# PaddlePaddle/Paddle3D

Measured on AMD Instinct MI355X. Metric: scenes/sec CenterPoint-Pillars nuScenes 300k-pt sweeps, higher is better.
Workload: dtype f32

## Files before the change

include/paddle3d_amd.h:

```cpp
#ifndef PADDLE3D_AMD_H
#define PADDLE3D_AMD_H

#include <stddef.h>
#include <stdint.h>

#ifdef __cplusplus
extern "C" {
#endif

#define PD3_OK 0
#define PD3_EINVAL (-1)
#define PD3_EWORKSPACE (-2)
#define PD3_EUNSUPPORTED (-3)

int pd3_version(void);
const char *pd3_target_arch(void);

int pd3_selfcheck_lds_atomic_order(const uint32_t *addr, uint32_t *old, int blocks, int waves_per_block, int rounds,
                                   int table, void *stream);

size_t pd3_hard_voxelize_workspace(int batch, int64_t max_points, int num_point_dim,
                                   const float *voxel_size, const float *point_cloud_range,
                                   int max_num_points_in_voxel, int max_voxels);
int pd3_hard_voxelize(const float *points, const int32_t *num_points, int batch, int64_t max_points,
                      int num_point_dim, const float *voxel_size, const float *point_cloud_range,
                      int max_num_points_in_voxel, int max_voxels, float *voxels, int32_t *coords,
                      int32_t *num_points_per_voxel, int32_t *num_voxels, int32_t *coors_batched,
                      void *workspace, size_t workspace_bytes, void *stream);
int pd3_hard_voxelize_path(const float *points, const int32_t *num_points, int batch, int64_t max_points,
                           int num_point_dim, const float *voxel_size, const float *point_cloud_range,
                           int max_num_points_in_voxel, int max_voxels, float *voxels, int32_t *coords,
                           int32_t *num_points_per_voxel, int32_t *num_voxels, int32_t *coors_batched,
                           void *workspace, size_t workspace_bytes, void *stream, int path);

int64_t pd3_hard_voxelize_index_list_entries(int batch, int64_t max_points);
int pd3_hard_voxelize_index(const float *points, const int32_t *num_points, int batch, int64_t max_points,
                            int num_point_dim, const float *voxel_size, const float *point_cloud_range,
                            int max_num_points_in_voxel, int max_voxels, int32_t *vox_span, int32_t *point_list,
                            int32_t *coords, int32_t *num_points_per_voxel, int32_t *num_voxels,
                            int32_t *coors_batched, void *workspace, size_t workspace_bytes, void *stream);

int pd3_hard_voxelize_f64(const double *points, const int32_t *num_points, int batch, int64_t max_points,
                          int num_point_dim, const float *voxel_size, const float *point_cloud_range,
                          int max_num_points_in_voxel, int max_voxels, double *voxels, int32_t *coords,
                          int32_t *num_points_per_voxel, int32_t *num_voxels, int32_t *coors_batched,
                          void *workspace, size_t workspace_bytes, void *stream);

int pd3_dynamic_voxelize(const float *points, int64_t num_points, int num_point_dim, const float *voxel_size,
                         const float *point_cloud_range, int32_t *coors, void *stream);

size_t pd3_pointpillars_scatter_workspace(int batch, int ny, int nx);
int pd3_pointpillars_scatter(const float *voxel_features, const int32_t *coords,
                             int64_t num_pillars, int channels, int batch, int ny, int nx,
                             float *canvas, void *workspace, size_t workspace_bytes, void *stream);

int pd3_pointpillars_inverse_map(const int32_t *coords, int64_t num_pillars, int batch, int ny, int nx,
                                 int32_t *inv, void *stream);
int pd3_scatter_conv3x3_bias_relu(const float *voxel_features, const int32_t *inv, const float *w_packed,
                                  const float *bias, int batch, int cin, int cout, int ny, int nx, int stride,
                                  int relu, float *out, int out_w, void *stream);

size_t pd3_pillar_conv_rulebook_workspace(int batch, int ny, int nx, int stride);
int pd3_pillar_conv_rulebook(const int32_t *inverse_map, int batch, int ny, int nx, int stride, int32_t *nbr,
                             int32_t *out_cell, int32_t *cell_row, int32_t *n_out, int capacity, int32_t *order,
                             void *workspace, size_t workspace_bytes, void *stream);
int pd3_rows_to_dense_fill(const float *rows, const int32_t *cell_row, const float *fill, int batch, int channels, int h,
                           int w, float *out, void *stream);

int pd3_pillar_feature_net(const float *voxels, const int32_t *num_points, const int32_t *coors,
                           int64_t num_pillars, int max_points, int num_point_dim,
                           int voxel_center_dims, float vx, float vy, float vz, float x_offset,
                           float y_offset, float z_offset, const float *w1, const float *scale1,
                           const float *shift1, int c1, const float *w2, const float *scale2,
                           const float *shift2, int c2, float *out, void *stream);

int pd3_pillar_feature_net_path(const float *voxels, const int32_t *num_points, const int32_t *coors,
                                int64_t num_pillars, int max_points, int num_point_dim,
                                int voxel_center_dims, float vx, float vy, float vz, float x_offset,
                                float y_offset, float z_offset, const float *w1, const float *scale1,
                                const float *shift1, int c1, const float *w2, const float *scale2,
                                const float *shift2, int c2, float *out, int path, void *stream);

int pd3_pillar_feature_net_indexed(const float *points, int64_t points_per_frame, const int32_t *vox_span,
                                   const int32_t *point_list, int64_t list_stride, const int32_t *coors,
                                   int64_t num_pillars, int pillars_per_frame, int max_points, int num_point_dim,
                                   int voxel_center_dims, float vx, float vy, float vz, float x_offset,
                                   float y_offset, float z_offset, const float *w1, const float *scale1,
                                   const float *shift1, int c1, const float *w2, const float *scale2,
                                   const float *shift2, int c2, float *out, void *stream);

int pd3_voxel_mean(const float *voxels, const int32_t *num_points, int64_t num_voxels,
                   int max_points, int num_point_dim, float *out, void *stream);

size_t pd3_nms_workspace(int num_boxes);
int pd3_nms_bev(const float *boxes, int num_boxes, float nms_overlap_thresh, int32_t *keep,
                int32_t *num_to_keep, void *workspace, size_t workspace_bytes, void *stream);
int pd3_nms_normal(const float *boxes, int num_boxes, float nms_overlap_thresh, int32_t *keep,
                   int32_t *num_to_keep, void *workspace, size_t workspace_bytes, void *stream);
int pd3_boxes_iou_bev(const float *boxes_a, int num_a, const float *boxes_b, int num_b,
                      float *ans_iou, void *stream);
int pd3_boxes_overlap_bev(const float *boxes_a, int num_a, const float *boxes_b, int num_b,
                          float *ans_overlap, void *stream);
int pd3_libm_eval(int op, const float *x, const float *y, float *out, int64_t n, void *stream);

size_t pd3_centerpoint_postprocess_workspace(int batch, int num_tasks, int feat_h, int feat_w,
                                             int nms_pre_max_size, int nms_post_max_size);
int pd3_centerpoint_postprocess(const float *const *hm, const float *const *reg,
                                const float *const *height, const float *const *dim,
                                const float *const *vel, const float *const *rot, int batch,
                                int num_tasks, const int *hm_channels, int feat_h, int feat_w,
                                const float *voxel_size, const float *point_cloud_range,
                                const float *post_center_range, const int *label_offsets,
                                int down_ratio, float score_threshold, float nms_iou_threshold,
                                int nms_pre_max_size, int nms_post_max_size, int with_velocity,
                                float *out_bboxes, float *out_scores, int64_t *out_labels,
                                int32_t *out_count, void *workspace, size_t workspace_bytes,
                                void *stream);

int pd3_centerpoint_postprocess_strided(const float *const *hm, const float *const *reg,
                                const float *const *height, const float *const *dim,
                                const float *const *vel, const float *const *rot, int64_t head_batch_stride, int batch,
                                int num_tasks, const int *hm_channels, int feat_h, int feat_w,
                                const float *voxel_size, const float *point_cloud_range,
                                const float *post_center_range, const int *label_offsets,
                                int down_ratio, float score_threshold, float nms_iou_threshold,
                                int nms_pre_max_size, int nms_post_max_size, int with_velocity,
                                float *out_bboxes, float *out_scores, int64_t *out_labels,
                                int32_t *out_count, void *workspace, size_t workspace_bytes,
                                void *stream, int selection);
int pd3_centerpoint_postprocess_records(const float *const *hm, const float *const *reg,
                                        const float *const *height, const float *const *dim,
                                        const float *const *vel, const float *const *rot,
                                        int64_t head_batch_stride, int batch, int num_tasks,
                                        const int *hm_channels, int feat_h, int feat_w, const float *voxel_size,
                                        const float *point_cloud_range, const float *post_center_range,
                                        const int *label_offsets, int down_ratio, float score_threshold,
                                        float nms_iou_threshold, int nms_pre_max_size, int nms_post_max_size,
                                        int with_velocity, float *out_bboxes, float *out_scores,
                                        int64_t *out_labels, int32_t *out_count, float *out_records,
                                        int max_per_img, void *workspace, size_t workspace_bytes, void *stream);

size_t pd3_bevdet_postprocess_workspace(int batch, int num_tasks, const int *task_classes, int feat_h, int feat_w,
                                        int max_num);
int pd3_bevdet_postprocess(const float *const *heatmap, const float *const *reg, const float *const *height,
                           const float *const *dim, const float *const *rot, const float *const *vel, int batch,
                           int num_tasks, const int *task_classes, int feat_h, int feat_w, const int *nms_type,
                           const float *nms_thr, const double *min_radius, const float *rescale_factors,
                           int max_num, int pre_max_size, int post_max_size, float score_threshold, int norm_bbox,
                           const float *post_center_range, const float *post_center_limit_range,
                           const float *pc_range, const float *voxel_size, float out_size_factor,
// ... 310 lines not shown
```

paddle3d_amd/_lib.py:

```python
from __future__ import annotations

import ctypes as C
import os
from functools import lru_cache

_HERE = os.path.dirname(os.path.abspath(__file__))
LIB_PATH = os.path.join(_HERE, "lib", "libpaddle3d_amd.so")

c_f32p = C.c_void_p
c_i32p = C.c_void_p

_SIGNATURES = {
    "pd3_version": (C.c_int, []),
    "pd3_target_arch": (C.c_char_p, []),
    "pd3_hard_voxelize_workspace": (C.c_size_t, [C.c_int, C.c_int64, C.c_int, C.c_void_p, C.c_void_p,
                                                 C.c_int, C.c_int]),
    "pd3_hard_voxelize": (C.c_int, [C.c_void_p, C.c_void_p, C.c_int, C.c_int64, C.c_int, C.c_void_p,
                                    C.c_void_p, C.c_int, C.c_int, C.c_void_p, C.c_void_p, C.c_void_p,
                                    C.c_void_p, C.c_void_p, C.c_void_p, C.c_size_t, C.c_void_p]),
    "pd3_hard_voxelize_f64": (C.c_int, [C.c_void_p, C.c_void_p, C.c_int, C.c_int64, C.c_int, C.c_void_p,
                                    C.c_void_p, C.c_int, C.c_int, C.c_void_p, C.c_void_p, C.c_void_p,
                                    C.c_void_p, C.c_void_p, C.c_void_p, C.c_size_t, C.c_void_p]),
    "pd3_hard_voxelize_path": (C.c_int, [C.c_void_p, C.c_void_p, C.c_int, C.c_int64, C.c_int, C.c_void_p,
                                         C.c_void_p, C.c_int, C.c_int, C.c_void_p, C.c_void_p, C.c_void_p,
# ... 98 lines not shown
    "pd3_gather_gemm_f16": (C.c_int, [C.c_void_p, C.c_void_p, C.c_void_p, C.c_int, C.c_int, C.c_int, C.c_int,
                                      C.c_void_p, C.c_void_p, C.c_void_p, C.c_void_p, C.c_void_p, C.c_int, C.c_void_p,
                                      C.c_void_p, C.c_int, C.c_int, C.c_int, C.c_void_p]),
    "pd3_sparse_tile_order_entries": (C.c_int64, [C.c_int]),
    "pd3_sparse_tile_order": (C.c_int, [C.c_void_p, C.c_void_p, C.c_int, C.c_int, C.c_void_p, C.c_void_p]),
    "pd3_sparse_plan_workspace": (C.c_size_t, [C.c_int]),
    "pd3_sparse_conv_outputs_workspace": (C.c_size_t, [C.c_int] + [C.c_void_p] * 4),
    "pd3_sparse_sort_coords": (C.c_int, [C.c_void_p, C.c_int, C.c_int, C.c_void_p, C.c_void_p, C.c_void_p,
                                         C.c_void_p, C.c_void_p, C.c_size_t, C.c_void_p]),
    "pd3_sparse_conv_outputs": (C.c_int, [C.c_void_p, C.c_void_p, C.c_int, C.c_int, C.c_void_p, C.c_void_p,
                                          C.c_void_p, C.c_void_p, C.c_void_p, C.c_void_p, C.c_int, C.c_void_p,
                                          C.c_size_t, C.c_void_p]),
    "pd3_sparse_rulebook_workspace": (C.c_size_t, [C.c_int, C.c_void_p]),
    "pd3_sparse_rulebook": (C.c_int, [C.c_void_p, C.c_void_p, C.c_int, C.c_void_p, C.c_void_p, C.c_int, C.c_int,
                                      C.c_void_p, C.c_void_p, C.c_void_p, C.c_void_p, C.c_int, C.c_void_p,
                                      C.c_void_p, C.c_void_p, C.c_size_t, C.c_void_p]),
    "pd3_sparse_to_dense": (C.c_int, [C.c_void_p, C.c_void_p, C.c_void_p, C.c_int, C.c_int, C.c_int,
                                      C.c_void_p, C.c_void_p, C.c_void_p]),
    "pd3_selfcheck_lds_atomic_order": (C.c_int, [C.c_void_p, C.c_void_p, C.c_int, C.c_int, C.c_int, C.c_int,
                                                 C.c_void_p]),
    "pd3_conv3x3_f16_bias_relu": (C.c_int, [C.c_void_p, C.c_void_p, C.c_void_p, C.c_int, C.c_int, C.c_int, C.c_int,
                                            C.c_int, C.c_int, C.c_void_p, C.c_int, C.c_int, C.c_void_p]),
    "pd3_f32_nchw_to_f16_nhwc": (C.c_int, [C.c_void_p, C.c_int, C.c_int, C.c_int, C.c_int, C.c_void_p, C.c_void_p]),
    "pd3_conv3x3_f16_bias_relu_dual": (C.c_int, [C.c_void_p, C.c_void_p, C.c_void_p, C.c_int, C.c_int, C.c_int, C.c_int,
                                                 C.c_int, C.c_int, C.c_void_p, C.c_void_p, C.c_int, C.c_void_p]),
    "pd3_conv3x3_s2_f16_bias_relu": (C.c_int, [C.c_void_p, C.c_void_p, C.c_void_p, C.c_int, C.c_int, C.c_int, C.c_int,
                                               C.c_int, C.c_int, C.c_void_p, C.c_void_p]),
    "pd3_scatter_conv3x3_s2_f16_bias_relu": (C.c_int, [C.c_void_p, C.c_void_p, C.c_void_p, C.c_void_p, C.c_int, C.c_int,
                                                       C.c_int, C.c_int, C.c_int, C.c_int, C.c_void_p, C.c_int,
                                                       C.c_void_p]),
    "pd3_grouped_conv3x3_small_f16": (C.c_int, [C.c_void_p, C.c_void_p, C.c_void_p, C.c_int, C.c_int, C.c_int, C.c_int,
                                                C.c_int, C.c_int, C.c_void_p, C.c_int, C.c_int, C.c_void_p]),
    "pd3_grouped_conv3x3_small_f16_gm": (C.c_int, [C.c_void_p, C.c_void_p, C.c_void_p, C.c_int, C.c_int, C.c_int, C.c_int,
                                                   C.c_int, C.c_int, C.c_void_p, C.c_int, C.c_int, C.c_void_p]),
    "pd3_stable_argsort_workspace": (C.c_size_t, [C.c_int64, C.c_uint32]),
    "pd3_stable_argsort": (C.c_int, [C.c_void_p, C.c_int64, C.c_int, C.c_uint32, C.c_void_p, C.c_void_p, C.c_size_t,
                                     C.c_void_p]),
    "pd3_conv3x3_winograd43_pp_bias_relu": (C.c_int, [C.c_void_p, C.c_void_p, C.c_void_p, C.c_int, C.c_int, C.c_int,
                                                       C.c_int, C.c_int, C.c_int, C.c_int, C.c_void_p, C.c_void_p]),
    "pd3_conv3x3_winograd43_pp_trace": (C.c_int, [C.c_void_p, C.c_void_p, C.c_void_p, C.c_int, C.c_int, C.c_int, C.c_int,
                                                  C.c_int, C.c_int, C.c_void_p, C.c_void_p, C.c_void_p]),
    "pd3_merge_sweeps_workspace": (C.c_size_t, [C.c_int64]),
    "pd3_merge_sweeps": (C.c_int, [C.c_void_p, C.c_void_p, C.c_int, C.c_int, C.c_int, C.c_void_p, C.c_void_p,
                                   C.c_void_p, C.c_int, C.c_float, C.c_void_p, C.c_void_p, C.c_void_p, C.c_size_t,
                                   C.c_void_p]),
    "pd3_dynamic_voxelize": (C.c_int, [C.c_void_p, C.c_int64, C.c_int, C.c_void_p, C.c_void_p, C.c_void_p, C.c_void_p]),
    "pd3_conv3x3_bias_relu": (C.c_int, [C.c_void_p, C.c_void_p, C.c_void_p, C.c_int, C.c_int, C.c_int, C.c_int,
                                        C.c_int, C.c_int, C.c_int, C.c_int, C.c_void_p, C.c_int, C.c_void_p]),
    "pd3_conv3x3_winograd_bias_relu": (C.c_int, [C.c_void_p, C.c_void_p, C.c_void_p, C.c_int, C.c_int, C.c_int,
                                                 C.c_int, C.c_int, C.c_int, C.c_void_p, C.c_void_p]),
    "pd3_conv3x3_winograd43_bias_relu": (C.c_int, [C.c_void_p, C.c_void_p, C.c_void_p, C.c_int, C.c_int, C.c_int,
                                                   C.c_int, C.c_int, C.c_int, C.c_int, C.c_void_p, C.c_int,
                                                   C.c_void_p]),
    "pd3_patch_conv_bias_relu": (C.c_int, [C.c_void_p, C.c_void_p, C.c_void_p, C.c_int, C.c_int, C.c_int, C.c_int,
                                           C.c_int, C.c_int, C.c_int, C.c_int, C.c_void_p, C.c_int, C.c_int,
                                           C.c_void_p]),
    "pd3_patch_conv_x3_bias_relu": (C.c_int, [C.c_void_p, C.c_void_p, C.c_void_p, C.c_int, C.c_int, C.c_int, C.c_int,
                                              C.c_int, C.c_int, C.c_int, C.c_int, C.c_void_p, C.c_int, C.c_int,
                                              C.c_void_p]),
    "pd3_conv3x3_s2_x3_bias_relu": (C.c_int, [C.c_void_p, C.c_void_p, C.c_void_p, C.c_int, C.c_int, C.c_int, C.c_int,
                                              C.c_int, C.c_int, C.c_int, C.c_void_p, C.c_int, C.c_void_p]),
    "pd3_winograd43_input_transform_floats": (C.c_size_t, [C.c_int] * 4),
    "pd3_winograd43_input_transform": (C.c_int, [C.c_void_p, C.c_int, C.c_int, C.c_int, C.c_int, C.c_int, C.c_void_p,
                                                 C.c_void_p]),
    "pd3_conv3x3_winograd43_ppv_bias_relu": (C.c_int, [C.c_void_p, C.c_void_p, C.c_void_p, C.c_int, C.c_int, C.c_int,
                                                       C.c_int, C.c_int, C.c_int, C.c_int, C.c_void_p, C.c_void_p]),
    "pd3_ssd_postprocess_workspace": (C.c_size_t, [C.c_int] * 7),
    "pd3_ssd_postprocess": (C.c_int, [C.c_void_p, C.c_int64, C.c_int, C.c_int, C.c_int, C.c_int, C.c_int, C.c_int,
                                      C.c_int, C.c_int, C.c_int, C.c_void_p, C.c_void_p, C.c_void_p, C.c_int64,
                                      C.c_int, C.c_int, C.c_float, C.c_float, C.c_void_p, C.c_float, C.c_int, C.c_int,
                                      C.c_void_p, C.c_void_p, C.c_void_p, C.c_void_p, C.c_void_p, C.c_size_t,
                                      C.c_void_p, C.c_int]),
    "pd3_pointpillars_inverse_map": (C.c_int, [C.c_void_p, C.c_int64, C.c_int, C.c_int, C.c_int, C.c_void_p,
                                               C.c_void_p]),
    "pd3_scatter_conv3x3_bias_relu": (C.c_int, [C.c_void_p, C.c_void_p, C.c_void_p, C.c_void_p, C.c_int, C.c_int,
                                                C.c_int, C.c_int, C.c_int, C.c_int, C.c_int, C.c_void_p, C.c_int,
                                                C.c_void_p]),
    "pd3_pillar_conv_rulebook_workspace": (C.c_size_t, [C.c_int] * 4),
    "pd3_pillar_conv_rulebook": (C.c_int, [C.c_void_p, C.c_int, C.c_int, C.c_int, C.c_int, C.c_void_p, C.c_void_p,
                                           C.c_void_p, C.c_void_p, C.c_int, C.c_void_p, C.c_void_p, C.c_size_t,
                                           C.c_void_p]),
    "pd3_rows_to_dense_fill": (C.c_int, [C.c_void_p, C.c_void_p, C.c_void_p, C.c_int, C.c_int, C.c_int, C.c_int,
                                         C.c_void_p, C.c_void_p]),
    "pd3_bevdet_postprocess_workspace": (C.c_size_t, [C.c_int, C.c_int, C.c_void_p, C.c_int, C.c_int, C.c_int]),
    "pd3_bevdet_postprocess": (C.c_int, [C.c_void_p] * 6 + [C.c_int, C.c_int, C.c_void_p, C.c_int, C.c_int,
                                         C.c_void_p, C.c_void_p, C.c_void_p, C.c_void_p, C.c_int, C.c_int,
                                         C.c_int, C.c_float, C.c_int, C.c_void_p, C.c_void_p, C.c_void_p,
                                         C.c_void_p, C.c_float, C.c_void_p, C.c_void_p, C.c_void_p, C.c_void_p,
                                         C.c_void_p, C.c_size_t, C.c_void_p]),
    "pd3_circle_nms_workspace": (C.c_size_t, [C.c_int]),
    "pd3_circle_nms": (C.c_int, [C.c_void_p, C.c_int, C.c_double, C.c_void_p, C.c_void_p, C.c_void_p, C.c_size_t,
                                 C.c_void_p]),
    "pd3_bevdet4d_align": (C.c_int, [C.c_void_p, C.c_void_p] + [C.c_int] * 6 + [C.c_void_p] * 12),
    "pd3_grouped_conv3x3_small": (C.c_int, [C.c_void_p, C.c_void_p, C.c_void_p, C.c_int, C.c_int, C.c_int, C.c_int,
                                            C.c_int, C.c_int, C.c_void_p, C.c_void_p]),
    "pd3_grouped_conv3x3_small_slice": (C.c_int, [C.c_void_p, C.c_void_p, C.c_void_p, C.c_int, C.c_int, C.c_int,
                                                  C.c_int, C.c_int, C.c_int, C.c_void_p, C.c_int, C.c_int,
                                                  C.c_void_p]),
}

SYMBOLS = tuple(_SIGNATURES)

_SIGNATURES_ROI = {
    "pd3_voxel_pool": (C.c_int, [C.c_void_p] * 8 + [C.c_int] * 7 + [C.c_float] + [C.c_int] * 5 + [C.c_void_p] * 2),
    "pd3_roi_grid_points": (C.c_int, [C.c_void_p, C.c_int64, C.c_int, C.c_int] + [C.c_void_p] * 3 + [C.c_int] +
                            [C.c_void_p] * 3),
    "pd3_rcnn_decode_boxes": (C.c_int, [C.c_void_p, C.c_void_p, C.c_int64, C.c_void_p, C.c_void_p]),
    "pd3_class_agnostic_nms_workspace": (C.c_size_t, [C.c_int, C.c_int64, C.c_int]),
    "pd3_class_agnostic_nms": (C.c_int, [C.c_void_p, C.c_void_p, C.c_int, C.c_int64, C.c_int, C.c_int, C.c_float,
                                         C.c_void_p, C.c_int, C.c_float, C.c_int] + [C.c_void_p] * 5 +
                               [C.c_size_t, C.c_void_p]),
}

SYMBOLS_ROI = tuple(_SIGNATURES_ROI)

_SIGNATURES_HEAD = {
    "pd3_grouped_conv3x3_small_counts_slice": (C.c_int, [C.c_void_p, C.c_void_p, C.c_void_p, C.c_int, C.c_int, C.c_int,
                                                         C.c_int, C.c_void_p, C.c_int, C.c_int, C.c_void_p, C.c_int,
                                                         C.c_int, C.c_void_p]),
}

SYMBOLS_HEAD = tuple(_SIGNATURES_HEAD)

_SIGNATURES_PVRCNN = {
    "pd3_stack_sa_pool": (C.c_int, [C.c_void_p] * 11 + [C.c_int] * 5 + [C.c_float, C.c_int] + [C.c_void_p] * 2),
    "pd3_bev_interpolate": (C.c_int, [C.c_void_p, C.c_void_p, C.c_int64] + [C.c_int] * 4 + [C.c_float] * 5 +
                            [C.c_void_p] * 2),
}

SYMBOLS_PVRCNN = tuple(_SIGNATURES_PVRCNN)

_CADDN_GRID = [C.c_int] * 3 + [C.c_void_p] * 2 + [C.c_int, C.c_double, C.c_double]
_CADDN_IN = [C.c_void_p] * 5 + [C.c_int] * 5 + _CADDN_GRID
_SIGNATURES_CADDN = {
    "pd3_frustum_grid": (C.c_int, [C.c_void_p] * 3 + [C.c_int] + _CADDN_GRID + [C.c_int] + [C.c_void_p] * 2),
    "pd3_frustum_to_voxel_workspace": (C.c_size_t, [C.c_int] * 5),
    "pd3_frustum_to_voxel": (C.c_int, _CADDN_IN + [C.c_void_p, C.c_void_p, C.c_size_t, C.c_void_p]),
    "pd3_frustum_to_bev_workspace": (C.c_size_t, [C.c_int] * 7),
    "pd3_frustum_to_bev": (C.c_int, _CADDN_IN + [C.c_void_p] * 3 + [C.c_int, C.c_void_p, C.c_void_p, C.c_size_t,
                                                                    C.c_void_p]),
}

SYMBOLS_CADDN = tuple(_SIGNATURES_CADDN)

_SIGNATURES_BEVFORMER = {
    "pd3_bevformer_point_sampling": (C.c_int, [C.c_void_p] * 3 + [C.c_int] * 6 + [C.c_void_p] * 5),
    "pd3_bevformer_sca": (C.c_int, [C.c_void_p] * 7 + [C.c_int] * 9 + [C.c_void_p] * 2),
    "pd3_bevformer_tsa": (C.c_int, [C.c_void_p] * 6 + [C.c_int] * 7 + [C.c_void_p] * 2),
}

SYMBOLS_BEVFORMER = tuple(_SIGNATURES_BEVFORMER)

_SIGNATURES_BEVFORMER_DEC = {
    "pd3_mha_forward": (C.c_int, [C.c_void_p] * 3 + [C.c_int] * 5 + [C.c_float] + [C.c_void_p] * 2),
    "pd3_bevformer_dec_ca": (C.c_int, [C.c_void_p] * 6 + [C.c_int] * 8 + [C.c_void_p] * 2),
    "pd3_nms_free_decode": (C.c_int, [C.c_void_p] * 3 + [C.c_int] * 5 + [C.c_double, C.c_int] + [C.c_void_p] * 5),
}

SYMBOLS_BEVFORMER_DEC = tuple(_SIGNATURES_BEVFORMER_DEC)

_SIGNATURES_PETR = {
    "pd3_mha_stream_forward": (C.c_int, [C.c_void_p] * 4 + [C.c_int] * 5 + [C.c_float] + [C.c_void_p] * 2),
    "pd3_petr_coords3d": (C.c_int, [C.c_void_p] + [C.c_int] * 6 + [C.c_double, C.c_void_p, C.c_int] + [C.c_void_p] * 4),
}

SYMBOLS_PETR = tuple(_SIGNATURES_PETR)
# ... 44 lines not shown
```

paddle3d_amd/ops/conv.py:

```python
from __future__ import annotations

import ctypes

import torch

from ._common import check, lib, ptr, require_gpu, stream_ptr

__all__ = ["pack_conv3x3_weight", "conv3x3_bias_relu", "supported", "pitch4", "pack_grouped_weight", "grouped_conv3x3_small",
           "grouped_small_supported", "winograd_supported", "pack_winograd_weight", "conv3x3_winograd_bias_relu",
           "patch_mode", "patch_supported", "pack_patch_weight", "patch_conv_bias_relu",
           "patch_x3_supported", "pack_patch_weight_x3", "patch_conv_x3_bias_relu", "split_bf16x3",
           "conv3x3_s2_x3_supported", "pack_conv3x3_s2_x3_weight", "conv3x3_s2_x3_bias_relu",
           "winograd43_input_transform", "conv3x3_winograd43_ppv_bias_relu",
           "winograd43_supported", "winograd43_tile", "pack_winograd43_weight", "conv3x3_winograd43_bias_relu",
           "WINOGRAD43_PP_MIN_CIN", "winograd43_pp_supported", "pack_winograd43_lane_weight", "conv3x3_winograd43_pp_bias_relu",
           "f16_supported", "f16_tile", "pack_conv3x3_f16_weight", "conv3x3_f16_bias_relu", "to_f16_nhwc",
           "pack_grouped_weight_f16", "grouped_conv3x3_small_f16", "conv3x3_f16_bias_relu_dual",
           "s2_f16_supported", "conv3x3_s2_f16_bias_relu", "scatter_conv_s2_f16_supported",
           "scatter_conv3x3_s2_f16_bias_relu", "scatter_conv_sparse_supported", "scatter_conv3x3_sparse"]


def pitch4(w: int) -> int:
    return (int(w) + 3) // 4 * 4


def supported(cin: int, cout: int, h: int, w: int, stride: int = 1) -> bool:
    return stride in (1, 2) and cin % 8 == 0 and cout % 64 == 0 and h % stride == 0 and w % stride == 0


def pack_conv3x3_weight(weight: torch.Tensor) -> torch.Tensor:
    cout, cin = weight.shape[:2]
    assert weight.shape[2:] == (3, 3) and cout % 64 == 0 and cin % 8 == 0
    w = weight.reshape(cout // 64, 64, cin // 8, 4, 2, 9).permute(0, 2, 3, 5, 4, 1)
    return w.reshape(cout // 64, cin // 8, 72, 64).contiguous()


def conv3x3_bias_relu(x: torch.Tensor, w_packed: torch.Tensor, bias, cout: int, relu: bool = True,
                      stride: int = 1, out: torch.Tensor | None = None, w_valid: int | None = None) -> torch.Tensor:
    xx = require_gpu(x, "conv3x3_bias_relu")
    n, cin, h, w = xx.shape
    wv = w if w_valid is None else int(w_valid)
    if out is None:
        out = torch.empty((n, cout, h // stride, pitch4(wv // stride)), dtype=torch.float32, device=xx.device)
    check(lib().pd3_conv3x3_bias_relu(ptr(xx), ptr(w_packed), ptr(bias), n, cin, cout, h, w, wv, int(stride),
                                      int(bool(relu)), ptr(out), int(out.shape[3]), stream_ptr(xx.device)),
          "conv3x3_bias_relu")
    return out


def scatter_conv_supported(cin: int, cout: int, ny: int, nx: int, stride: int) -> bool:
    return stride == 2 and cin % 8 == 0 and cout % 64 == 0 and ny % 2 == 0 and nx % 2 == 0


def scatter_conv3x3_bias_relu(canvas, w_packed: torch.Tensor, bias, cout: int, relu: bool = True) -> torch.Tensor:
    f, inv = canvas.features, canvas.inv
    n, cin, ny, nx = canvas.shape
    wo = pitch4(nx // 2)
    out = torch.empty((n, cout, ny // 2, wo), dtype=torch.float32, device=f.device)
    check(lib().pd3_scatter_conv3x3_bias_relu(ptr(f), ptr(inv), ptr(w_packed), ptr(bias), n, cin, cout, ny, nx, 2,
                                              int(bool(relu)), ptr(out), wo, stream_ptr(f.device)),
          "scatter_conv3x3_bias_relu")
    return out


def scatter_conv_sparse_supported(cin: int, cout: int, ny: int, nx: int, stride: int) -> bool:
    ho, wo = (ny - 1) // stride + 1, (nx - 1) // stride + 1
    return stride == 2 and cin % 16 == 0 and cout in (64, 128) and wo % 4 == 0 and (ho * wo) % 4 == 0


def scatter_conv3x3_sparse(canvas, weight: torch.Tensor, bias: torch.Tensor, packed=None, relu: bool = True):
    from . import sparse_conv3d as sp
    from ._common import workspace

    f, inv = canvas.features, canvas.inv
    n, cin, ny, nx = canvas.shape
    cout = int(weight.shape[0])
    ho, wo = (ny - 1) // 2 + 1, (nx - 1) // 2 + 1
    cap = n * ho * wo
    dev = f.device
    L = lib()
    nbr = torch.empty((cap, 9), dtype=torch.int32, device=dev)
    out_cell = torch.empty((cap,), dtype=torch.int32, device=dev)
    cell_row = torch.empty((n, ho * wo), dtype=torch.int32, device=dev)
    n_out = torch.empty((1,), dtype=torch.int32, device=dev)
    ws = workspace(L.pd3_pillar_conv_rulebook_workspace(n, ny, nx, 2), dev)
    order = torch.empty((int(L.pd3_sparse_tile_order_entries(cap)),), dtype=torch.int32, device=dev)
    check(L.pd3_pillar_conv_rulebook(ptr(inv), n, ny, nx, 2, ptr(nbr), ptr(out_cell), ptr(cell_row), ptr(n_out), cap,
                                     ptr(order), ptr(ws), ws.numel(), stream_ptr(dev)), "pillar_conv_rulebook")
    idx = sp.SparseIndices(None, nbr, cap, (1, ho, wo), 9, order, n_out)
    if packed is None:
        packed = sp.pack_weight_bf16x3(weight.permute(2, 3, 1, 0).reshape(1, 3, 3, cin, cout).contiguous())
    rows = sp.features_bf16x3(f, idx, packed, cin, cout, bias, None, None, None, relu)
    fill = torch.relu(bias) if relu else bias
    out = torch.empty((n, cout, ho, wo), dtype=torch.float32, device=dev)
    check(L.pd3_rows_to_dense_fill(ptr(rows), ptr(cell_row), ptr(fill.contiguous()), n, cout, ho, wo, ptr(out),
                                   stream_ptr(dev)), "rows_to_dense_fill")
    return out, packed


def winograd_supported(cin: int, cout: int, h: int, w: int) -> bool:
    return cin % 8 == 0 and cout % 32 == 0 and w % 4 == 0


def pack_winograd_weight(weight: torch.Tensor) -> torch.Tensor:
    cout, cin = weight.shape[:2]
    assert weight.shape[2:] == (3, 3) and cout % 32 == 0 and cin % 8 == 0
    g = torch.tensor([[1.0, 0.0, 0.0], [0.5, 0.5, 0.5], [0.5, -0.5, 0.5], [0.0, 0.0, 1.0]], dtype=torch.float64,
                     device=weight.device)
    u = torch.einsum("ij,ocjk,lk->ocil", g, weight.double(), g).float()
    u = u.reshape(cout // 32, 2, 16, cin // 8, 8, 16).permute(0, 3, 1, 4, 2, 5)
    return u.contiguous()


def conv3x3_winograd_bias_relu(x: torch.Tensor, u_packed: torch.Tensor, bias, cout: int, relu: bool = True,
                               out: torch.Tensor | None = None) -> torch.Tensor:
    xx = require_gpu(x, "conv3x3_winograd_bias_relu")
    n, cin, h, w = xx.shape
    if out is None:
        out = torch.empty((n, cout, h, w), dtype=torch.float32, device=xx.device)
    check(lib().pd3_conv3x3_winograd_bias_relu(ptr(xx), ptr(u_packed), ptr(bias), n, cin, cout, h, w,
                                               int(bool(relu)), ptr(out), stream_ptr(xx.device)),
          "conv3x3_winograd_bias_relu")
    return out


def winograd43_supported(cin: int, cout: int, h: int, w: int) -> bool:
    return cin % 4 == 0 and cout % 32 == 0


def winograd43_tile(cout: int) -> int:
    return 64 if cout % 64 == 0 else 32


def _winograd43_u(weight: torch.Tensor) -> torch.Tensor:
    g = torch.tensor([[1 / 4, 0, 0], [-1 / 6, -1 / 6, -1 / 6], [-1 / 6, 1 / 6, -1 / 6], [1 / 24, 1 / 12, 1 / 6],
                      [1 / 24, -1 / 12, 1 / 6], [0, 0, 1]], dtype=torch.float64, device=weight.device)
    return torch.einsum("ij,ocjk,lk->ocil", g, weight.double(), g).float()


def pack_winograd43_weight(weight: torch.Tensor, tile: int | None = None) -> torch.Tensor:
    cout, cin = weight.shape[:2]
    t = winograd43_tile(cout) if tile is None else tile
    assert weight.shape[2:] == (3, 3) and cout % t == 0 and cin % 4 == 0 and t in (32, 64)
    u = _winograd43_u(weight).reshape(cout // t, t // 16, 16, cin // 4, 4, 36).permute(0, 3, 1, 4, 2, 5)
    return u.contiguous()


def conv3x3_winograd43_bias_relu(x: torch.Tensor, u_packed: torch.Tensor, bias, cout: int, relu: bool = True,
                                 out: torch.Tensor | None = None, w_valid: int | None = None) -> torch.Tensor:
    xx = require_gpu(x, "conv3x3_winograd43_bias_relu")
    n, cin, h, w = xx.shape
    tile = 16 * u_packed.shape[2]
    if out is None:
        out = torch.empty((n, cout, h, w), dtype=torch.float32, device=xx.device)
    check(lib().pd3_conv3x3_winograd43_bias_relu(ptr(xx), ptr(u_packed), ptr(bias), n, cin, cout, h, w,
                                                 w if w_valid is None else int(w_valid), int(bool(relu)), ptr(out),
                                                 tile, stream_ptr(xx.device)),
          "conv3x3_winograd43_bias_relu")
    return out


def patch_mode(weight: torch.Tensor, stride: int, transpose: bool):
    k = weight.shape[2]
    if weight.shape[2] != weight.shape[3] or k != stride:
        return None
    if k == 1:
        return 1
    if k == 2:
        return 2 if transpose else 0
    if k == 4 and transpose:
        return 3
    return None


def patch_supported(mode: int, cin: int, cout: int, h: int, w: int) -> bool:
    if mode == 0:
        return h % 4 == 0 and w % 4 == 0 and (cin * 4) % 16 == 0 and cout % 64 == 0
    if (h * w) % 4 or cin % 16:
# ... 336 lines not shown
```

Measured before the change: 2288.

## Add specialized 64x64 pillar sparse conv kernel with pipelined bf16x3 MFMA

Adds a dedicated HIP kernel for the first sparse pillar conv when cin and cout are both 64. It is a persistent kernel with XCD-aware tile scheduling that double-buffers per-tap weights in LDS via DMA and prefetches neighbor feature rows two steps ahead. It also skips taps that no row in the tile uses, and runs bf16x3 split MFMA to keep f32-level accuracy. The Python path routes to it by default and caches the relu(bias) fill tensor, at the cost of a large hand-scheduled kernel whose correctness rests on subtle mask and barrier logic.

```diff
diff --git a/include/paddle3d_amd.h b/include/paddle3d_amd.h
--- a/include/paddle3d_amd.h
+++ b/include/paddle3d_amd.h
@@ -66,6 +66,11 @@
                              void *workspace, size_t workspace_bytes, void *stream);
 int pd3_rows_to_dense_fill(const float *rows, const int32_t *cell_row, const float *fill, int batch, int channels, int h,
                            int w, float *out, void *stream);
+
+int pd3_pillar_conv_features_grid_entries(int capacity);
+int pd3_pillar_conv_features_bf16x3(const float *in_feats, const int32_t *nbr, const int32_t *order, const int32_t *n_out,
+                                    int capacity, int kernel_volume, int cin, int cout, const void *weight_packed,
+                                    const float *bias, int relu, float *out, int grid_blocks, void *stream);
 
 int pd3_pillar_feature_net(const float *voxels, const int32_t *num_points, const int32_t *coors,
                            int64_t num_pillars, int max_points, int num_point_dim,
diff --git a/paddle3d_amd/_lib.py b/paddle3d_amd/_lib.py
--- a/paddle3d_amd/_lib.py
+++ b/paddle3d_amd/_lib.py
@@ -204,6 +204,9 @@
                                            C.c_void_p]),
     "pd3_rows_to_dense_fill": (C.c_int, [C.c_void_p, C.c_void_p, C.c_void_p, C.c_int, C.c_int, C.c_int, C.c_int,
                                          C.c_void_p, C.c_void_p]),
+    "pd3_pillar_conv_features_grid_entries": (C.c_int, [C.c_int]),
+    "pd3_pillar_conv_features_bf16x3": (C.c_int, [C.c_void_p] * 4 + [C.c_int] * 4 +
+                                        [C.c_void_p, C.c_void_p, C.c_int, C.c_void_p, C.c_int, C.c_void_p]),
     "pd3_bevdet_postprocess_workspace": (C.c_size_t, [C.c_int, C.c_int, C.c_void_p, C.c_int, C.c_int, C.c_int]),
     "pd3_bevdet_postprocess": (C.c_int, [C.c_void_p] * 6 + [C.c_int, C.c_int, C.c_void_p, C.c_int, C.c_int,
                                          C.c_void_p, C.c_void_p, C.c_void_p, C.c_void_p, C.c_int, C.c_int,
diff --git a/paddle3d_amd/csrc/pillar_gemm_x3.hip b/paddle3d_amd/csrc/pillar_gemm_x3.hip
--- /dev/null
+++ b/paddle3d_amd/csrc/pillar_gemm_x3.hip
@@ -0,0 +1,362 @@
+#include "../../include/paddle3d_amd.h"
+#include "bf16x3.hpp"
+#include "common.hpp"
+#include <algorithm>
+
+namespace pd3 {
+
+constexpr int kPgLine = 72;
+constexpr int kPgWFetches = 28;
+constexpr int kPgWBytes = kPgWFetches * 1024;
+constexpr int kPgTapBytes = 3 * 64 * 64 * 2;
+constexpr int kPgWindow = 8192;
+
+typedef int pg_i32x4 __attribute__((ext_vector_type(4), aligned(4)));
+struct PgNbr {
+  pg_i32x4 lo, hi;
+  int last;
+};
+
+struct PgArgs {
+  const float* in;
+  const int32_t* nbr;
+  const int32_t* order;
+  const int* n_out_dev;
+  const __bf16* wpk;
+  const float* bias;
+  float* out;
+  int cap, relu;
+};
+
+constexpr int kPgWaves = 4;
+constexpr int kPgRows = 32 * kPgWaves;
+constexpr size_t kPgLds = (size_t)2 * kPgWBytes + (size_t)(2 * 9 + 3) * kPgRows * sizeof(int) + 48 * sizeof(uint32_t) +
+                          64 * sizeof(float);
+
+__global__ __launch_bounds__(64 * kPgWaves, 2) void pillar_gemm_x3_kernel(PgArgs a) {
+  constexpr int WAVES = kPgWaves;
+  constexpr int T = kPgRows;
+  constexpr int FPW = kPgWFetches / WAVES;
+  static_assert(FPW * WAVES == kPgWFetches, "every wave sends the same number of weight fetches");
+  constexpr int PW = kPgWindow / T;
+  extern __shared__ __attribute__((aligned(16))) unsigned char pg_smem[];
+  unsigned char* Ws = pg_smem;
+  int* nbs = reinterpret_cast<int*>(pg_smem + 2 * kPgWBytes);
+  int* rows_l = nbs + 2 * 9 * T;
+  uint32_t* masks_l = reinterpret_cast<uint32_t*>(rows_l + 3 * T);
+  float* bias_s = reinterpret_cast<float*>(masks_l + 48);
+  const int tid = threadIdx.x, lane = lane_id(), wave = __builtin_amdgcn_readfirstlane(wave_id());
+  const int l31 = lane & 31, kh = lane >> 5;
+  const int n_out = a.n_out_dev ? min(*a.n_out_dev, a.cap) : a.cap;
+  const int ntiles = (n_out + T - 1) / T;
+  const int64_t vtot = ((int64_t)ntiles + 8 * PW - 1) / (8 * PW) * (8 * PW);
+
+  int fv = 0;
+  auto next_tile = [&]() -> int {
+    while (true) {
+      const int64_t v = (int64_t)blockIdx.x + (int64_t)fv * gridDim.x;
+      if (v >= vtot) return -1;
+      ++fv;
+      const int xcd = (int)(v & 7), slot = (int)(v >> 3);
+      const int w = slot / PW, pos = (int)((slot % PW + 23ll * w) % PW);
+      const int t = (w * 8 + xcd) * PW + pos;
+      if (t < ntiles) return t;
+    }
+  };
+  auto load_order = [&](int tile) -> int {
+    const int32_t* p = a.order ? a.order + ((int64_t)max(tile, 0) * T + min(tid, T - 1)) : a.nbr;
+    return *p;
+  };
+  auto order_row = [&](int tile, int raw) -> int {
+    const int64_t s = (int64_t)max(tile, 0) * T + tid;
+    const int r = a.order ? raw : (int)min(s, (int64_t)n_out);
+    return tile >= 0 && tid < T && r >= 0 && r < n_out ? r : -1;
+  };
+  auto load_nbr = [&](int row, PgNbr& nb) {
+    const int32_t* p = a.nbr + (int64_t)max(row, 0) * 9;
+    nb.lo = *reinterpret_cast<const pg_i32x4*>(p);
+    nb.hi = *reinterpret_cast<const pg_i32x4*>(p + 4);
+    nb.last = p[8];
+  };
+  auto write_idx = [&](int ti, int row, const PgNbr& nb, bool exists) {
+    const int s2 = ti & 1, s3 = ti % 3;
+    if (tid < T) {
+      uint32_t m = 0;
+#pragma unroll
+      for (int k = 0; k < 9; ++k) {
+        const int v = row >= 0 ? (k < 4 ? nb.lo[k & 3] : k < 8 ? nb.hi[k & 3] : nb.last) : -1;
+        nbs[(s2 * 9 + k) * T + tid] = v;
+        m |= v >= 0 ? 1u << k : 0u;
+      }
+      rows_l[s3 * T + tid] = row;
+#pragma unroll
+      for (int d = 1; d < 32; d <<= 1) m |= (uint32_t)__shfl_xor((int)m, d, kWave);
+      if (l31 == 0) masks_l[s3 * 16 + (tid >> 5)] = m;
+    }
+    if (tid == 0) masks_l[s3 * 16 + 15] = exists ? 1u : 0u;
+  };
+
+  unsigned wvoff[FPW];
+#pragma unroll
+  for (int j = 0; j < FPW; ++j) {
+    const int e = (wave * FPW + j) * 64 + lane;
+    const int line = e / 9, q = e - line * 9;
+    const int p = line >> 6, co = line & 63;
+    wvoff[j] = (q < 8 && line < 192) ? (unsigned)((((q >> 2) * 3 + p) * 64 + co) * 64 + (q & 3) * 16) : kPxOob;
+  }
+  auto dma_w = [&](int k, unsigned char* dst) {
+    const unsigned so = __builtin_amdgcn_readfirstlane((unsigned)k * (unsigned)kPgTapBytes);
+#pragma unroll
+    for (int j = 0; j < FPW; ++j) {
+      const int f = wave * FPW + j;
+      px_dma(a.wpk, 9u * kPgTapBytes, dst + f * 1024, wvoff[j], so);
+    }
+  };
+
+  if (tid < 64) bias_s[tid] = a.bias ? a.bias[tid] : 0.f;
+  int ordn, ordt, rowv = -1;
+  PgNbr nbv;
+  bool exv = false;
+  {
+    const int t0 = next_tile(), t1 = next_tile();
+    ordt = next_tile();
+    if (t0 < 0) return;
+    const int o0 = load_order(t0), o1 = load_order(t1);
+    ordn = load_order(ordt);
+    const int r0 = order_row(t0, o0), r1 = order_row(t1, o1);
+    PgNbr nb0, nb1;
+    load_nbr(r0, nb0);
+    load_nbr(r1, nb1);
+    write_idx(0, r0, nb0, true);
+    write_idx(1, r1, nb1, t1 >= 0);
+  }
+  nbv.lo = nbv.hi = pg_i32x4{-1, -1, -1, -1};
+  nbv.last = -1;
+  __syncthreads();
+
+  struct Cur {
+    int ti, k;
+    uint32_t rest, blk;
+    bool first;
+  };
+  auto enter = [&](Cur& c) {
+    const uint32_t* ml = masks_l + (c.ti % 3) * 16;
+    c.first = true;
+    c.rest = c.blk = 0u;
+    c.k = -1;
+    if (!__builtin_amdgcn_readfirstlane((int)ml[15])) return;
+    uint32_t m = 0;
+#pragma unroll
+    for (int w = 0; w < WAVES; ++w) m |= ml[w];
+    m = (uint32_t)__builtin_amdgcn_readfirstlane((int)m);
+    if (!(m & (m - 1))) m |= (m & 1u) ? 2u : 1u;
+    if (!(m & (m - 1))) m |= 2u;
+    c.k = __builtin_ctz(m);
+    c.rest = m & (m - 1);
+    c.blk = (uint32_t)__builtin_amdgcn_readfirstlane((int)ml[wave]);
+  };
+  auto advance = [&](Cur& c) {
+    if (c.k < 0) return;
+    if (c.rest) {
+      c.k = __builtin_ctz(c.rest);
+      c.rest &= c.rest - 1;
+      c.first = false;
+    } else {
+      ++c.ti;
+      enter(c);
+    }
+  };
+
+  px_f32x16 acc[2];
+#pragma unroll
+  for (int i = 0; i < 2; ++i)
+#pragma unroll
+    for (int r = 0; r < 16; ++r) acc[i][r] = 0.f;
+  px_b8 bp[4][3];
+  px_f32x4 raw_a[4][2], raw_b[4][2];
+  int j_a, j_b;
+
+  auto fetch_b = [&](const Cur& c, px_f32x4 (&dst)[4][2], int& jv) {
+    const bool on = c.k >= 0 && ((c.blk >> c.k) & 1u);
+    const int j = on ? nbs[((c.ti & 1) * 9 + max(c.k, 0)) * T + wave * 32 + l31] : -1;
+    jv = j;
+    const px_f32x4* src = reinterpret_cast<const px_f32x4*>(a.in + (int64_t)max(j, 0) * 64 + kh * 16);
+#pragma unroll
+    for (int cc = 0; cc < 2; ++cc)
+#pragma unroll
+      for (int s = 0; s < 2; ++s) {
+        dst[cc * 2 + s][0] = src[cc * 8 + 2 * s];
+        dst[cc * 2 + s][1] = src[cc * 8 + 2 * s + 1];
+      }
+  };
+  auto split_b = [&](const px_f32x4 (&src)[4][2], int jv) {
+    const bool live = jv >= 0;
+#pragma unroll
+    for (int s = 0; s < 4; ++s) {
+      px_f32x4 lo4 = src[s][0], hi4 = src[s][1];
+#pragma unroll
+      for (int e = 0; e < 4; ++e) {
+        lo4[e] = live ? lo4[e] : 0.f;
+        hi4[e] = live ? hi4[e] : 0.f;
+      }
+      px_split(lo4, hi4, bp[s][0], bp[s][1], bp[s][2]);
+    }
+  };
+  auto epilogue = [&](int ti) {
+    const int row = rows_l[(ti % 3) * T + wave * 32 + l31];
+    px_f32x4 o[2][4];
+#pragma unroll
+    for (int i = 0; i < 2; ++i) {
+#pragma unroll
+      for (int q = 0; q < 4; ++q) {
+        const int co = i * 32 + 8 * q + 4 * kh;
+        float v[4];
+#pragma unroll
+        for (int e = 0; e < 4; ++e) v[e] = acc[i][4 * q + e];
+        if (a.bias) {
+          const px_f32x4 b4 = *reinterpret_cast<const px_f32x4*>(bias_s + co);
+#pragma unroll
+          for (int e = 0; e < 4; ++e) v[e] += b4[e];
+        }
+        if (a.relu) {
+#pragma unroll
+          for (int e = 0; e < 4; ++e) v[e] = fmaxf(v[e], 0.f);
+        }
+        o[i][q] = px_f32x4{v[0], v[1], v[2], v[3]};
+      }
+    }
+    if (row >= 0) {
+      px_f32x4* dst = reinterpret_cast<px_f32x4*>(a.out + (int64_t)row * 64 + 4 * kh);
+#pragma unroll
+      for (int i = 0; i < 2; ++i)
+#pragma unroll
+        for (int q = 0; q < 4; ++q) dst[i * 8 + 2 * q] = o[i][q];
+    }
+#pragma unroll
+    for (int i = 0; i < 2; ++i)
+#pragma unroll
+      for (int r = 0; r < 16; ++r) acc[i][r] = 0.f;
+  };
+
+  Cur c0, c1, c2;
+  c0.ti = 0;
+  enter(c0);
+  c1 = c0;
+  advance(c1);
+  c2 = c1;
+  advance(c2);
+  int buf = 0;
+  dma_w(c0.k, Ws);
+  asm volatile("" ::: "memory");
+  fetch_b(c0, raw_a, j_a);
+  fetch_b(c1, raw_b, j_b);
+  if ((c0.blk >> c0.k) & 1u) split_b(raw_a, j_a);
+  PX_VMCNT(8);
+  px_lds_barrier();
+
+  auto step = [&](px_f32x4 (&near)[4][2], int& jn, px_f32x4 (&far)[4][2], int& jf) {
+    const bool last = c0.rest == 0u;
+    if (c0.first) {
+      rowv = order_row(ordt, ordn);
+      exv = ordt >= 0;
+      load_nbr(rowv, nbv);
+      ordt = next_tile();
+      ordn = load_order(ordt);
+    }
+    asm volatile("" ::: "memory");
+    dma_w(c1.k >= 0 ? c1.k : c0.k, Ws + (buf ^ 1) * kPgWBytes);
+    asm volatile("" ::: "memory");
+    fetch_b(c2, far, jf);
+    asm volatile("" ::: "memory");
+    if ((c0.blk >> c0.k) & 1u) {
+      const __bf16* wl = reinterpret_cast<const __bf16*>(Ws + buf * kPgWBytes) + l31 * kPgLine + kh * 8;
+#pragma unroll
+      for (int i = 0; i < 2; ++i) {
+#pragma unroll
+        for (int s = 0; s < 4; ++s) {
+          px_b8 av[3];
+#pragma unroll
+          for (int p = 0; p < 3; ++p) av[p] = *reinterpret_cast<const px_b8*>(wl + (p * 64 + i * 32) * kPgLine + s * 16);
+          acc[i] = __builtin_amdgcn_mfma_f32_32x32x16_bf16(av[0], bp[s][2], acc[i], 0, 0, 0);
+          acc[i] = __builtin_amdgcn_mfma_f32_32x32x16_bf16(av[2], bp[s][0], acc[i], 0, 0, 0);
+          acc[i] = __builtin_amdgcn_mfma_f32_32x32x16_bf16(av[1], bp[s][1], acc[i], 0, 0, 0);
+          acc[i] = __builtin_amdgcn_mfma_f32_32x32x16_bf16(av[0], bp[s][1], acc[i], 0, 0, 0);
+          acc[i] = __builtin_amdgcn_mfma_f32_32x32x16_bf16(av[1], bp[s][0], acc[i], 0, 0, 0);
+          acc[i] = __builtin_amdgcn_mfma_f32_32x32x16_bf16(av[0], bp[s][0], acc[i], 0, 0, 0);
+        }
+      }
+    }
+    if (c1.k >= 0 && ((c1.blk >> c1.k) & 1u)) split_b(near, jn);
+    PX_VMCNT(8);
+    if (last) {
+      epilogue(c0.ti);
+      write_idx(c0.ti + 2, rowv, nbv, exv);
+    }
+    px_lds_barrier();
+    buf ^= 1;
+    c0 = c1;
+    c1 = c2;
+    advance(c2);
+  };
+  while (true) {
+    step(raw_b, j_b, raw_a, j_a);
+    if (c0.k < 0) break;
+    step(raw_a, j_a, raw_b, j_b);
+    if (c0.k < 0) break;
+  }
+  PX_VMCNT(0);
+}
+
+static inline int pg_cu_count() {
+  static std::mutex mu;
+  static std::vector<int> cus;
+  int dev = 0;
+  if (hipGetDevice(&dev) != hipSuccess) return 0;
+  std::lock_guard<std::mutex> lock(mu);
+  if ((int)cus.size() <= dev) cus.resize(dev + 1, 0);
+  if (cus[dev] == 0) {
+    int n = 0;
+    if (hipDeviceGetAttribute(&n, hipDeviceAttributeMultiprocessorCount, dev) != hipSuccess || n <= 0) return 0;
+    cus[dev] = n;
+  }
+  return cus[dev];
+}
+
+}
+
+using namespace pd3;
+
+extern "C" int pd3_pillar_conv_features_grid_entries(int capacity) {
+  if (capacity <= 0) return 0;
+  const int cus = pg_cu_count();
+  if (cus <= 0) return 0;
+  const long long want = 4LL * cus;
+  const long long items = sp_window_grid(ceil_div(capacity, kPgRows), kPgWindow / kPgRows);
+  return (int)std::min(want, items);
+}
+
+extern "C" int pd3_pillar_conv_features_bf16x3(const float* in_feats, const int32_t* nbr, const int32_t* order,
+                                               const int32_t* n_out, int capacity, int kernel_volume, int cin, int cout,
+                                               const void* weight_packed, const float* bias, int relu, float* out,
+                                               int grid_blocks, void* stream) {
+  if (!in_feats || !nbr || !weight_packed || !out || capacity <= 0 || kernel_volume <= 0 || cin <= 0 || cout <= 0 ||
+      grid_blocks < 0)
+    return PD3_EINVAL;
+  if (kernel_volume != 9 || cin != 64 || cout != 64) return PD3_EUNSUPPORTED;
+  if (reinterpret_cast<uintptr_t>(in_feats) % 16 != 0 || reinterpret_cast<uintptr_t>(weight_packed) % 16 != 0 ||
+      reinterpret_cast<uintptr_t>(out) % 16 != 0 || (bias && reinterpret_cast<uintptr_t>(bias) % 16 != 0) ||
+      reinterpret_cast<uintptr_t>(nbr) % 4 != 0 || (order && reinterpret_cast<uintptr_t>(order) % 4 != 0) ||
+      (n_out && reinterpret_cast<uintptr_t>(n_out) % 4 != 0))
+    return PD3_EINVAL;
+  int grid = grid_blocks;
+  if (grid == 0) {
+    grid = pd3_pillar_conv_features_grid_entries(capacity);
+    if (grid <= 0) return PD3_EINVAL;
+  }
+  grid = (int)std::min<long long>(grid, sp_window_grid(ceil_div(capacity, kPgRows), kPgWindow / kPgRows));
+  PgArgs a{in_feats, nbr, order, n_out, static_cast<const __bf16*>(weight_packed), bias, out, capacity, relu ? 1 : 0};
+  const hipError_t e = pd3_max_dynamic_lds(reinterpret_cast<const void*>(pillar_gemm_x3_kernel), (int)kPgLds);
+  if (e != hipSuccess) return (int)e;
+  pillar_gemm_x3_kernel<<<(unsigned)grid, 64 * kPgWaves, kPgLds, static_cast<hipStream_t>(stream)>>>(a);
+  return launch_status();
+}
diff --git a/paddle3d_amd/ops/conv.py b/paddle3d_amd/ops/conv.py
--- a/paddle3d_amd/ops/conv.py
+++ b/paddle3d_amd/ops/conv.py
@@ -17,7 +17,8 @@
            "f16_supported", "f16_tile", "pack_conv3x3_f16_weight", "conv3x3_f16_bias_relu", "to_f16_nhwc",
            "pack_grouped_weight_f16", "grouped_conv3x3_small_f16", "conv3x3_f16_bias_relu_dual",
            "s2_f16_supported", "conv3x3_s2_f16_bias_relu", "scatter_conv_s2_f16_supported",
-           "scatter_conv3x3_s2_f16_bias_relu", "scatter_conv_sparse_supported", "scatter_conv3x3_sparse"]
+           "scatter_conv3x3_s2_f16_bias_relu", "scatter_conv_sparse_supported", "scatter_conv3x3_sparse", "pillar_kernel_supported",
+           "SparseFirstPacked"]
 
 
 def pitch4(w: int) -> int:
@@ -66,6 +67,25 @@
 def scatter_conv_sparse_supported(cin: int, cout: int, ny: int, nx: int, stride: int) -> bool:
     ho, wo = (ny - 1) // stride + 1, (nx - 1) // stride + 1
     return stride == 2 and cin % 16 == 0 and cout in (64, 128) and wo % 4 == 0 and (ho * wo) % 4 == 0
+
+
+PILLAR_KERNEL = True
+
+
+class SparseFirstPacked:
+
+    def __init__(self, weight: torch.Tensor):
+        self.weight = weight
+        self.fill = {}
+
+    def fill_for(self, bias: torch.Tensor, relu: bool) -> torch.Tensor:
+        if relu not in self.fill:
+            self.fill[relu] = (torch.relu(bias) if relu else bias.clone()).contiguous()
+        return self.fill[relu]
+
+
+def pillar_kernel_supported(cin: int, cout: int) -> bool:
+    return cin == 64 and cout == 64
 
 
 def scatter_conv3x3_sparse(canvas, weight: torch.Tensor, bias: torch.Tensor, packed=None, relu: bool = True):
@@ -87,13 +107,25 @@
     order = torch.empty((int(L.pd3_sparse_tile_order_entries(cap)),), dtype=torch.int32, device=dev)
     check(L.pd3_pillar_conv_rulebook(ptr(inv), n, ny, nx, 2, ptr(nbr), ptr(out_cell), ptr(cell_row), ptr(n_out), cap,
                                      ptr(order), ptr(ws), ws.numel(), stream_ptr(dev)), "pillar_conv_rulebook")
-    idx = sp.SparseIndices(None, nbr, cap, (1, ho, wo), 9, order, n_out)
     if packed is None:
         packed = sp.pack_weight_bf16x3(weight.permute(2, 3, 1, 0).reshape(1, 3, 3, cin, cout).contiguous())
-    rows = sp.features_bf16x3(f, idx, packed, cin, cout, bias, None, None, None, relu)
-    fill = torch.relu(bias) if relu else bias
+    if not isinstance(packed, SparseFirstPacked):
+        packed = SparseFirstPacked(packed)
+    if PILLAR_KERNEL and pillar_kernel_supported(cin, cout):
+        ff = require_gpu(f, "scatter_conv3x3_sparse")
+        if ff.shape[1] != cin or packed.weight.numel() != 3 * 9 * cin * cout:
+            raise RuntimeError("scatter_conv3x3_sparse: weight / feature shapes do not match")
+        bb = None if bias is None else require_gpu(bias, "scatter_conv3x3_sparse")
+        rows = torch.empty((cap, cout), dtype=torch.float32, device=dev)
+        check(L.pd3_pillar_conv_features_bf16x3(ptr(ff), ptr(nbr), ptr(order) if sp.TILE_ORDER else None, ptr(n_out), cap,
+                                                9, cin, cout, ptr(packed.weight), ptr(bb), int(bool(relu)), ptr(rows),
+                                                0, stream_ptr(dev)), "pillar_conv_features_bf16x3")
+    else:
+        idx = sp.SparseIndices(None, nbr, cap, (1, ho, wo), 9, order, n_out)
+        rows = sp.features_bf16x3(f, idx, packed.weight, cin, cout, bias, None, None, None, relu)
+    fill = packed.fill_for(bias, bool(relu))
     out = torch.empty((n, cout, ho, wo), dtype=torch.float32, device=dev)
-    check(L.pd3_rows_to_dense_fill(ptr(rows), ptr(cell_row), ptr(fill.contiguous()), n, cout, ho, wo, ptr(out),
+    check(L.pd3_rows_to_dense_fill(ptr(rows), ptr(cell_row), ptr(fill), n, cout, ho, wo, ptr(out),
                                    stream_ptr(dev)), "rows_to_dense_fill")
     return out, packed
 
```

After: 2303 (median of 6 runs). Within noise of the previous version (+0.7%).
